# NonStopEagle137/Visual-Inertial-Odometry-MSCKF-Stereo

Measured on AMD Instinct MI355X. Metric: EKF measurement updates/sec at 30 cam-states x 200 features; ATE RMSE vs ref, higher is better.
Workload: dtype f32/f64; 1 GPU; batched EKF measurement update, 30 cam-states x 200 features, 2048 filters/GPU, triangulation + jacobian + gating + information assembly + Kalman, no row cap; cam_states=30, features=200, filters_per_gpu=2048, parallelism=replicas1

## Files before the change

visual-inertial-odometry-msckf-stereo_amd/csrc/msckf_api.hip:

```cpp
#include <hip/hip_runtime.h>

#include <algorithm>
#include <cmath>
#include <cstdio>
#include <cstring>
#include <string>
#include <vector>

#include "../../include/msckf_hip.h"
#include "msckf_common.h"
#include "msckf_launch.h"
#include "msckf_subbatch.h"

using namespace msckf;

static thread_local std::string g_err;

#define FAIL(code, ...)                                  \
    do {                                                 \
        char _b[512];                                    \
        snprintf(_b, sizeof(_b), __VA_ARGS__);           \
        g_err = _b;                                      \
        return (code);                                   \
    } while (0)
// ... 152 lines not shown
namespace {

template <typename T>
Params<T> make_params(const msckf_ctx* c) {
    Params<T> p{};
    const msckf_config_t& k = c->cfg;
    p.sigma2 = (T)k.observation_noise;
    p.qc_gyro = (T)k.gyro_noise;
    p.qc_gbias = (T)k.gyro_bias_noise;
    p.qc_acc = (T)k.acc_noise;
    p.qc_abias = (T)k.acc_bias_noise;
    for (int i = 0; i < 9; ++i) p.R01[i] = (T)k.R_cam0_cam1[i];
    for (int i = 0; i < 3; ++i) p.t01[i] = (T)k.t_cam0_cam1[i];
    p.huber = (T)k.huber_epsilon;
    p.precision = (T)k.estimation_precision;
    p.damping = (T)k.initial_damping;
    p.outer_max = k.outer_loop_max_iteration;
    p.inner_max = k.inner_loop_max_iteration;
    return p;
}

template <typename T>
DevState<T> dev_state(msckf_ctx* c, int b0 = 0, int nb = -1) {
    DevState<T> s;
    s.P = reinterpret_cast<T*>(c->P.p) + (size_t)b0 * c->Dmax * c->Dmax;
    s.imu = reinterpret_cast<T*>(c->imu.p) + (size_t)b0 * IMU_STRIDE;
    s.cams = reinterpret_cast<T*>(c->cams.p) + (size_t)b0 * c->Nmax * CAM_STRIDE;
    s.ncams = c->ncams.p + b0;
    s.B = nb < 0 ? c->B - b0 : nb;
    s.Nmax = c->Nmax;
    s.Dmax = c->Dmax;
    return s;
}

template <typename T>
UpdWs<T> upd_ws(msckf_ctx* c, int b0 = 0) {
    UpdWs<T> w;
    const size_t b = (size_t)b0, C = (size_t)c->Cmax;
    w.Cmax = c->Cmax;
    w.Cp = (c->Cmax + 15) & ~15;
    w.wk_stride = kalman_global_ws_doubles(c->Cmax);
    w.Hthin = reinterpret_cast<KT*>(c->Hthin.p) + b * C * (C + 1);
    w.dx = reinterpret_cast<KT*>(c->dx.p) + b * (c->Dmax + C);
    w.info = c->info.p + 4 * b;
    w.Lc = reinterpret_cast<KT*>(c->Lc.p) + b * w.Cp * w.Cp;
    w.afail = c->afail.p + b;
    w.Vi = reinterpret_cast<KT*>(c->Vi.p) + b * 24 * w.Cp;
    w.Sii = reinterpret_cast<KT*>(c->Sii.p) + b * 24 * 24;
    w.G = reinterpret_cast<KT*>(c->G.p) + b * C * (C + 1);
    w.Tm = reinterpret_cast<KT*>(c->Tm.p) + b * C * (C + 1);
    w.W = reinterpret_cast<KT*>(c->W.p) + b * (c->Dmax + 1) * w.Cp;
    w.Wk = c->Wk.p ? reinterpret_cast<KT*>(c->Wk.p) + b * w.wk_stride : nullptr;
    w.s2 = (double)(T)c->cfg.observation_noise;
    return w;
}

template <typename T>
FeatBatch<T> feat_batch(msckf_ctx* c) {
    FeatBatch<T> f;
    f.nf = c->nf;
    f.feat_filter = c->feat_filter;
    f.feat_off = c->feat_off;
    f.obs_off = c->obs_off;
    f.obs_cam = c->obs_cam;
    f.obs_z = reinterpret_cast<const T*>(c->obs_z);
    f.chi2 = reinterpret_cast<const T*>(c->chi2);
    f.ysq_off = c->ysq_off;
    f.p_w = reinterpret_cast<T*>(c->p_w);
    f.valid = c->valid;
    f.obs_ws = reinterpret_cast<T*>(c->obs_ws.p);
    f.obs_ht = reinterpret_cast<T*>(c->obs_ht.p);
    f.obs_g = reinterpret_cast<double*>(c->obs_g.p);
    f.fqr = reinterpret_cast<double*>(c->fqr.p);
    f.gram = c->gram ? 1 : 0;
    f.compact = feature_needs_compact(c->maxM) ? 1 : 0;
    f.tau = reinterpret_cast<T*>(c->tau.p);
    f.ysq = reinterpret_cast<T*>(c->ysq.p);
    f.gamma = reinterpret_cast<T*>(c->gamma);
    f.accept = c->accept;
    f.include = c->include;
    f.row_off = c->row_off.p;
    return f;
}

template <typename T>
std::vector<T> to_T(const double* x, size_t n) {
    std::vector<T> v(n);
    for (size_t i = 0; i < n; ++i) v[i] = (T)x[i];
    return v;
}

template <typename T>
hipError_t upload(msckf_ctx* c, void* dst, const double* src, size_t n) {
    if (n == 0) return hipSuccess;
    unsigned char* h = nullptr;
    hipError_t e = c->up.get(n * sizeof(T), &h);
    if (e != hipSuccess) return e;
    T* v = reinterpret_cast<T*>(h);
    for (size_t i = 0; i < n; ++i) v[i] = (T)src[i];
    e = hipMemcpyAsync(dst, h, n * sizeof(T), hipMemcpyHostToDevice, c->stream);
    if (e != hipSuccess) return e;
    return c->up.mark(c->stream);
}

hipError_t upload_raw(msckf_ctx* c, void* dst, const void* src, size_t bytes) {
    if (bytes == 0) return hipSuccess;
// ... 1089 lines not shown
        t->reset();
    }
    return 0;
}

int msckf_set_profiling_stage(msckf_ctx_t* c, const char* stage) {
    if (!c) FAIL(-1, "null context");
    if (int r = sync_lanes(c)) return r;
    for (KernelTimer* t : {&c->timer, &c->timer1}) {
        t->on = stage != nullptr;
        t->only = stage ? stage : "";
        t->reset();
    }
    return 0;
}

int msckf_kernel_times(msckf_ctx_t* c, int max_k, double* ms_total, int32_t* launches, char* names_out,
                       int names_cap) {
    if (!c) FAIL(-1, "null context");
    if (int r = sync_lanes(c)) return r;
    int k = std::min<int>(max_k, (int)c->timer.names.size());
    std::string all;
    for (int i = 0; i < k; ++i) {
        ms_total[i] = c->timer.total_ms[i];
        for (size_t j = 0; j < c->timer1.names.size(); ++j)
            if (c->timer1.names[j] == c->timer.names[i]) ms_total[i] += c->timer1.total_ms[j];
        launches[i] = c->timer.launches[i];
        all += c->timer.names[i];
        all.push_back('\0');
    }
    if (names_out && names_cap > 0) {
        int n = std::min<int>(names_cap - 1, (int)all.size());
        std::memcpy(names_out, all.data(), n);
        names_out[n] = 0;
    }
    return k;
}

int msckf_debug_workspace(msckf_ctx_t* c, int which, double* out, size_t count) {
    if (!c || !out) FAIL(-1, "null argument");
    JOIN_LANES(c);
    const void* src = which == 0 ? c->Lc.p : which == 1 ? c->Vi.p : which == 2 ? c->Sii.p
                    : which == 3 ? c->G.p : which == 4 ? c->Tm.p : which == 5 ? c->W.p
                    : which == 6 ? (const void*)c->Hthin.p : which == 7 ? (const void*)c->afail.p : nullptr;
    if (!src) FAIL(-1, "unknown workspace %d", which);
    HIPSYNC(c, hipStreamSynchronize(c->stream));
    HIPC(hipMemcpy(out, src, count * sizeof(double), hipMemcpyDeviceToHost));
    return 0;
}

int msckf_debug_set_workspace(msckf_ctx_t* c, int which, const double* in, size_t count) {
    if (!c || !in) FAIL(-1, "null argument");
    JOIN_LANES(c);
    void* dst = which == 6 ? (void*)c->Hthin.p : nullptr;
    if (!dst) FAIL(-1, "unknown workspace %d", which);
    if (count * sizeof(double) > c->Hthin.cap) FAIL(-1, "%zu doubles exceed H_thin", count);
    HIPSYNC(c, hipStreamSynchronize(c->stream));
    HIPC(hipMemcpy(dst, in, count * sizeof(double), hipMemcpyHostToDevice));
    return 0;
}

int msckf_debug_lanes(msckf_ctx_t* c) {
    if (!c) FAIL(-1, "null context");
    return c->last_lanes;
}

int msckf_debug_kalman(msckf_ctx_t* c) {
    if (c) c->last_async = "msckf_debug_kalman";
    if (!c) FAIL(-1, "null context");
    JOIN_LANES(c);
    return DISPATCH(c, run_kalman_only, c);
}

}
```

visual-inertial-odometry-msckf-stereo_amd/csrc/msckf_common.h:

```cpp
#pragma once
#include <hip/hip_runtime.h>
#include <stdint.h>

namespace msckf {

constexpr int IMU_STRIDE = 48;
enum ImuField { I_Q = 0, I_P = 4, I_V = 7, I_BG = 10, I_BA = 13, I_QN = 16, I_PN = 20,
                I_VN = 23, I_RIC = 26, I_TCI = 35, I_G = 38, I_ALIAS = 41 };
constexpr int CAM_STRIDE = 12;
enum CamField { C_Q = 0, C_P = 4, C_QN = 7 };

constexpr int OBS_HX = 0, OBS_V = 24, OBS_W = 36, OBS_QR = 54, OBS_R = 58, OBS_WS = 62;
constexpr int OBS_HT = 0, OBS_RT = 18, OBS_HTS = 24;

constexpr int OBG_G = 0, OBG_DS = 18, OBG_UB = 39, OBG_CAM = 45, OBG_STRIDE = 46;
constexpr int FQR_X = 0, FQR_G = 6, FQR_FLAG = 9, FQR_STRIDE = 10;
constexpr double FQR_RMAX = 1e3, FQR_KAPPA = 1e4;

template <typename T>
struct Params {
    T sigma2;
    T qc_gyro, qc_gbias, qc_acc, qc_abias;
    T R01[9], t01[3];
    T huber, precision, damping;
// ... 2 lines not shown

template <typename T>
struct DevState {
    T* P;
    T* imu;
    T* cams;
    int* ncams;
    int B, Nmax, Dmax;
};

template <typename T>
struct FeatBatch {
    int nf;
    const int* feat_filter;
    const int* feat_off;
    const int* obs_off;
    const int* obs_cam;
    const T* obs_z;
    const T* chi2;
    const long long* ysq_off;
    T* p_w;
    uint8_t* valid;
    T* obs_ws;
    T* obs_ht;
    double* obs_g;
    double* fqr;
    int gram;
    int compact;
    T* tau;
    T* ysq;
    T* gamma;
    uint8_t* accept;
    uint8_t* include;
    int* row_off;
};

using KT = double;
template <typename T>
struct UpdWs {
    KT* Hthin;
    KT* dx;
    int* info;
    int Cmax;
    KT* Lc;
    KT* Vi;
    KT* Sii;
    KT* G;
    KT* Tm;
    KT* W;
    KT* Wk;
    int* afail;
    size_t wk_stride;
    int Cp;
    double s2;
};

template <typename T> __device__ __forceinline__ T dsqrt(T x) { return sqrt(x); }

template <typename T>
__device__ __forceinline__ void skew3(const T* v, T* S) {
    S[0] = 0;     S[1] = -v[2]; S[2] = v[1];
    S[3] = v[2];  S[4] = 0;     S[5] = -v[0];
    S[6] = -v[1]; S[7] = v[0];  S[8] = 0;
}

template <typename T>
__device__ __forceinline__ void quat_to_rot(const T* q_in, T* R) {
    T n = sqrt(q_in[0] * q_in[0] + q_in[1] * q_in[1] + q_in[2] * q_in[2] + q_in[3] * q_in[3]);
    T x = q_in[0] / n, y = q_in[1] / n, z = q_in[2] / n, w = q_in[3] / n;
    T v[3] = {x, y, z};
    T S[9];
    skew3(v, S);
    T a = 2 * w * w - 1, tw = 2 * w;
#pragma unroll
    for (int i = 0; i < 3; ++i)
#pragma unroll
        for (int j = 0; j < 3; ++j)
            R[3 * i + j] = (i == j ? a : T(0)) - tw * S[3 * i + j] + (2 * v[i]) * v[j];
}

template <typename T>
__device__ __forceinline__ void rot_to_quat(const T* R, T* q) {
    T t;
    if (R[8] < 0) {
        if (R[0] > R[4]) {
            t = 1 + R[0] - R[4] - R[8];
            q[0] = t; q[1] = R[1] + R[3]; q[2] = R[6] + R[2]; q[3] = R[5] - R[7];
        } else {
            t = 1 - R[0] + R[4] - R[8];
            q[0] = R[1] + R[3]; q[1] = t; q[2] = R[7] + R[5]; q[3] = R[6] - R[2];
        }
    } else {
        if (R[0] < -R[4]) {
            t = 1 - R[0] - R[4] + R[8];
            q[0] = R[2] + R[6]; q[1] = R[7] + R[5]; q[2] = t; q[3] = R[1] - R[3];
        } else {
            t = 1 + R[0] + R[4] + R[8];
            q[0] = R[5] - R[7]; q[1] = R[6] - R[2]; q[2] = R[1] - R[3]; q[3] = t;
        }
    }
    T n = sqrt(q[0] * q[0] + q[1] * q[1] + q[2] * q[2] + q[3] * q[3]);
    q[0] /= n; q[1] /= n; q[2] /= n; q[3] /= n;
}

template <typename T>
__device__ __forceinline__ void quat_mul(const T* a_in, const T* b_in, T* q) {
// ... 111 lines not shown
```

visual-inertial-odometry-msckf-stereo_amd/csrc/msckf_kalman.hip:

```cpp
#include "msckf_common.h"
#include "msckf_launch.h"
#include "msckf_rchol.h"

#include <stdlib.h>

namespace msckf {

constexpr int KW = 24;

__device__ __forceinline__ int round4(int x) { return (x + 3) & ~3; }


typedef double v4d __attribute__((ext_vector_type(4)));

constexpr double KALMAN_PIVOT_FLOOR = 1e-10;

template <typename T>
__device__ double diag_max(const T* M, int ld, int o, int n, double* lds) {
    double m = 0.0;
    for (int i = threadIdx.x; i < n; i += blockDim.x) m = fmax(m, (double)M[(size_t)(o + i) * (ld + 1)]);
    m = wave_max(m);
    if ((threadIdx.x & 63) == 0) lds[threadIdx.x >> 6] = m;
    __syncthreads();
    for (int w = 0; w < (int)(blockDim.x >> 6); ++w) m = fmax(m, lds[w]);
// ... 5 lines not shown
    return diag_max(P, ld, 21, C, lds) * KALMAN_PIVOT_FLOOR;
}
constexpr double T_FLOOR_NEG = 1e-9;

template <typename T, int NT, int TPL, bool RETRY = false>
__global__ void __launch_bounds__(NT) __attribute__((amdgpu_waves_per_eu(NT == 256 ? 2 : 1))) k_kal_a(DevState<T> st, UpdWs<T> ws) {
    extern __shared__ __attribute__((aligned(16))) unsigned char smem_raw[];
    const int b = blockIdx.x;
    if (RETRY && ws.afail[b] == 0) return;
    const int C = 6 * st.ncams[b], Cp = round4(C);
    const int nrow = (Cp + KW) / 4;
    const T* P = st.P + (size_t)b * st.Dmax * st.Dmax;
    const int ld = st.Dmax, Cpw = ws.Cp;
    KT* Lc = ws.Lc + (size_t)b * Cpw * Cpw;
    KT* Vi = ws.Vi + (size_t)b * KW * Cpw;
    KT* Sii = ws.Sii + (size_t)b * KW * KW;
    auto map = [&](int i) { return i < C ? 21 + i : (i < Cp ? -1 : (i < Cp + 21 ? i - Cp : -1)); };
    double shift = 0.0;
    auto load = [&](int i, int j) -> double {
        const int mi = map(i), mj = map(j);
        if (mi < 0 || mj < 0) return i == j ? 1.0 : 0.0;
        return (double)P[(size_t)mi * ld + mj] + (i == j && i < C ? shift : 0.0);
    };
    auto panel = [&](int r, int c0, double w0, double w1, double w2, double w3) {
        KT* dst = r < Cp ? Lc + (size_t)r * Cpw + c0 : Vi + (size_t)(r - Cp) * Cpw + c0;
        dst[0] = w0; dst[1] = w1; dst[2] = w2; dst[3] = w3;
    };
    auto trail = [&](int i, int j, double v) { Sii[(i - Cp) * KW + (j - Cp)] = v; };
    const double floor = pcc_pivot_floor(P, ld, C, reinterpret_cast<double*>(smem_raw));
    bool ok = false;
    for (int att = RETRY ? 1 : 0; att < (RETRY ? 3 : 1) && !ok; ++att) {
        if (att > 0) {
            shift = (att == 1 ? 1e-8 : 1e-6) * (floor / KALMAN_PIVOT_FLOOR);
            __syncthreads();
        }
        ok = rchol_core<NT, TPL>(nrow, nrow, Cp / 4, reinterpret_cast<double*>(smem_raw), load, panel, trail, floor);
    }
    if (threadIdx.x == 0) ws.afail[b] = ok ? 0 : 1;
}

template <typename T, int NT, int TPL>
__global__ void __launch_bounds__(NT) __attribute__((amdgpu_waves_per_eu(NT == 256 ? 2 : 1))) k_kal_c1(DevState<T> st, UpdWs<T> ws) {
    extern __shared__ __attribute__((aligned(16))) unsigned char smem_raw[];
    const int b = blockIdx.x;
    if (ws.info[4 * b] == 0) return;
    if (ws.afail[b]) {
        if (threadIdx.x == 0) ws.info[4 * b + 3] = -2;
        return;
    }
    const int C = 6 * st.ncams[b], Cp = round4(C), nTc = Cp / 4;
    const int ldt = ws.Cmax + 1;
    const KT* Tm = ws.Tm + (size_t)b * ws.Cmax * ldt;
    KT* L = ws.G + (size_t)b * ws.Cmax * ldt;
    auto load = [&](int i, int j) -> double {
        if (i >= C || j >= C) return i == j ? 1.0 : 0.0;
        return i >= j ? Tm[(size_t)i * ldt + j] : Tm[(size_t)j * ldt + i];
    };
    auto panel = [&](int r, int c0, double w0, double w1, double w2, double w3) {
        if (r >= C) return;
        KT* dst = L + (size_t)r * ldt;
        const double w[4] = {w0, w1, w2, w3};
#pragma unroll
        for (int q = 0; q < 4; ++q)
            if (c0 + q < C && c0 + q <= r) dst[c0 + q] = w[q];
    };
    auto trail = [](int, int, double) {};
    const double tmax = diag_max(Tm, ldt, 0, C, reinterpret_cast<double*>(smem_raw));
    const bool ok = rchol_core<NT, TPL>(nTc, nTc, nTc, reinterpret_cast<double*>(smem_raw), load, panel, trail, ws.s2,
                                        -T_FLOOR_NEG * tmax);
    if (!ok && threadIdx.x == 0) ws.info[4 * b + 3] = -1;
}

constexpr int C2S = 17;

template <typename T, int NW, int CT, int NTM>
__global__ void __launch_bounds__(64 * NW) k_kal_c2(DevState<T> st, UpdWs<T> ws) {
    extern __shared__ __attribute__((aligned(16))) unsigned char smem_raw[];
    constexpr int NT = 64 * NW;
    const int b = blockIdx.x;
    if (ws.info[4 * b] == 0 || ws.info[4 * b + 3] < 0) return;
    const int C = 6 * st.ncams[b], nT = (C + 15) / 16, E = 22 + C, nE = (E + 15) / 16;
    const int tid = threadIdx.x, lane = tid & 63, lc = lane & 15, lr = lane >> 4;
    const int wv = __builtin_amdgcn_readfirstlane(tid >> 6);
    const int ldt = ws.Cmax + 1, Cpw = ws.Cp, ldw = st.Dmax + 1;
    const KT* L = ws.G + (size_t)b * ws.Cmax * ldt;
    const KT* Tm = ws.Tm + (size_t)b * ws.Cmax * ldt;
    const KT* Lc = ws.Lc + (size_t)b * Cpw * Cpw;
    const KT* Vi = ws.Vi + (size_t)b * KW * Cpw;
    KT* Wt = ws.W + (size_t)b * (st.Dmax + 1) * Cpw;
    double* LI = reinterpret_cast<double*>(smem_raw);
    double* img = LI + NTM * 256;
    auto Lv = [&](int r, int k) -> double {
        if (r >= C || k >= C) return r == k ? 1.0 : 0.0;
        return k <= r ? L[(size_t)r * ldt + k] : 0.0;
    };
    for (int J = wv; J < nT; J += NW) {
        double* blk = img + wv * 272;
#pragma unroll
        for (int q = 0; q < 4; ++q) {
            const int e = lane + 64 * q, i = e >> 4, k = e & 15;
            blk[e] = Lv(16 * J + i, 16 * J + k);
        }
        __builtin_amdgcn_wave_barrier();
        __builtin_amdgcn_fence(__ATOMIC_ACQ_REL, "wavefront");
        if (lane < 16) blk[256 + lane] = 1.0 / blk[17 * lane];
        __builtin_amdgcn_wave_barrier();
        __builtin_amdgcn_fence(__ATOMIC_ACQ_REL, "wavefront");
        if (lane < 16) {
            double x[16];
#pragma unroll
            for (int i = 0; i < 16; ++i) {
                double sv = i == lane ? 1.0 : 0.0;
#pragma unroll
                for (int k = 0; k < i; ++k) sv -= k >= lane ? blk[16 * i + k] * x[k] : 0.0;
                x[i] = i < lane ? 0.0 : sv * blk[256 + i];
            }
            double* xj = LI + J * 256 + 16 * lane;
#pragma unroll
            for (int i = 0; i < 16; ++i) xj[i] = x[i];
        }
        __builtin_amdgcn_wave_barrier();
        __builtin_amdgcn_fence(__ATOMIC_ACQ_REL, "wavefront");
    }
    auto Xv = [&](int e, int j) -> double {
        if (j >= C) return 0.0;
        if (e < 21) return Vi[(size_t)e * Cpw + j];
        if (e < 21 + C) return j <= e - 21 ? Lc[(size_t)(e - 21) * Cpw + j] : 0.0;
        if (e == 21 + C) return Tm[(size_t)j * ldt + C];
        return 0.0;
    };
    v4d yk[CT][NTM];
    constexpr int PFN = (256 * (NTM - 1) + NT - 1) / NT;
    double pf[PFN];
    auto fetch = [&](int J) {
        const int w = 16 * J;
#pragma unroll
        for (int q = 0; q < PFN; ++q) {
            const int e = tid + NT * q, i = e / w, col = e - i * w;
            pf[q] = e < 16 * w ? -Lv(16 * J + i, col) : 0.0;
        }
    };
    constexpr int IMGB = 16 * NTM * C2S;
    auto imgJ = [&](int J) { return img + (J & 1) * IMGB; };
    auto put = [&](int J) {
        const int w = 16 * J;
        double* im = imgJ(J);
#pragma unroll
        for (int q = 0; q < PFN; ++q) {
            const int e = tid + NT * q, i = e / w, col = e - i * w;
            if (e < 16 * w) im[col * C2S + i] = pf[q];
        }
    };
    __syncthreads();
    if (nT > 1) fetch(1);
    v4d xn[CT];
#pragma unroll
    for (int t = 0; t < CT; ++t) {
        const int ct = wv + NW * t;
#pragma unroll
        for (int q = 0; q < 4; ++q) xn[t][q] = ct < nE ? Xv(16 * ct + lc, lr + 4 * q) : 0.0;
    }
#pragma unroll
    for (int J = 0; J < NTM; ++J) {
        if (J >= nT) continue;
        if (J > 0) put(J);
        __syncthreads();
        if (J + 1 < nT) fetch(J + 1);
#pragma unroll
        for (int t = 0; t < CT; ++t) {
            const int ct = wv + NW * t;
            if (ct >= nE) continue;
            v4d a0 = xn[t], a1 = v4d{0.0, 0.0, 0.0, 0.0};
            if (J + 1 < nT) {
#pragma unroll
                for (int q = 0; q < 4; ++q) xn[t][q] = Xv(16 * ct + lc, 16 * (J + 1) + lr + 4 * q);
            }
            const double* im = imgJ(J);
#pragma unroll
            for (int K = 0; K < J; ++K) {
#pragma unroll
                for (int kc = 0; kc < 4; ++kc) {
                    const double av = im[(16 * K + 4 * kc + lr) * C2S + lc];
                    if (K & 1) a1 = __builtin_amdgcn_mfma_f64_16x16x4f64(av, yk[t][K][kc], a1, 0, 0, 0);
                    else a0 = __builtin_amdgcn_mfma_f64_16x16x4f64(av, yk[t][K][kc], a0, 0, 0, 0);
                }
            }
            a0 += a1;
            v4d y = v4d{0.0, 0.0, 0.0, 0.0};
#pragma unroll
            for (int kc = 0; kc < 4; ++kc)
                y = __builtin_amdgcn_mfma_f64_16x16x4f64(LI[J * 256 + (4 * kc + lr) * 16 + lc], a0[kc], y, 0, 0, 0);
            yk[t][J] = y;
        }
    }
#pragma unroll
    for (int t = 0; t < CT; ++t) {
        const int ct = wv + NW * t, col = 16 * ct + lc;
        if (ct >= nE || col >= E) continue;
#pragma unroll
        for (int J = 0; J < NTM; ++J) {
            if (J >= nT) continue;
#pragma unroll
            for (int q = 0; q < 4; ++q) {
                const int k = 16 * J + lr + 4 * q;
                if (k < C) Wt[(size_t)k * ldw + col] = yk[t][J][q];
            }
        }
    }
}

constexpr int GNB = 64;

__host__ __device__ constexpr size_t gchol_c_off(int Cmax) { return (size_t)(Cmax + 21) * (Cmax + 21); }
template <int STAGE, typename T>
__device__ __forceinline__ bool gdims(const DevState<T>& st, const UpdWs<T>& ws, int b, KT*& A, int& nrow,
                                      int& ncol, int& nelim) {
    if (ws.info[4 * b] == 0 || ws.info[4 * b + 3] < 0) return false;
    const int C = 6 * st.ncams[b];
    A = ws.Wk + (size_t)b * ws.wk_stride + (STAGE == 0 ? 0 : gchol_c_off(ws.Cmax));
    if (STAGE == 0) { nrow = C + 21; ncol = C + 21; }
    else { nrow = C + 22 + C; ncol = C; }
    nelim = C;
    return true;
}

template <int STAGE, typename T>
__global__ void __launch_bounds__(64) k_gchol_diag(DevState<T> st, UpdWs<T> ws, int k) {
    const int b = blockIdx.x;
    KT* A;
    int nrow, ncol, nelim;
    if (!gdims<STAGE>(st, ws, b, A, nrow, ncol, nelim) || k >= nelim) return;
    const int ld = ncol, nb = nelim - k < GNB ? nelim - k : GNB;
    __shared__ double colj[2][GNB];
    __shared__ double lt[GNB * (GNB + 1) / 2];
    const int lane = threadIdx.x;
    double x[GNB];
    {
        const KT* src = A + (size_t)(k + lane) * ld + k;
#pragma unroll
        for (int j = 0; j < GNB; ++j) x[j] = (lane < nb && j <= lane) ? src[j] : (j == lane ? 1.0 : 0.0);
    }
    double floor = STAGE == 0 ? 0.0 : ws.s2, lo;
    if (STAGE == 0) {
        const T* P = st.P + (size_t)b * st.Dmax * st.Dmax;
        for (int i = lane; i < nelim; i += 64) floor = fmax(floor, (double)P[(size_t)(21 + i) * st.Dmax + 21 + i]);
        floor = wave_max(floor) * KALMAN_PIVOT_FLOOR;
        lo = -PIVOT_FLOOR_NEG * floor;
    } else {
        const int ldt = ws.Cmax + 1;
        const KT* Tm = ws.Tm + (size_t)b * ws.Cmax * ldt;
        double tmax = 0.0;
        for (int i = lane; i < nelim; i += 64) tmax = fmax(tmax, (double)Tm[(size_t)i * ldt + i]);
        lo = -T_FLOOR_NEG * wave_max(tmax);
    }
// ... 438 lines not shown
            if (ti[s] < 0) continue;
#pragma unroll
            for (int r = 0; r < 4; ++r) {
                const int i = 16 * ti[s] + lr + 4 * r, j = 16 * tj[s] + lc;
                if (i < C && j <= i) Tm[(size_t)i * ld + j] = acc[s][r] + (i == j ? s2 : 0.0);
            }
        }
        if (tid < C) Tm[(size_t)tid * ld + C] = ca;
    }
}

template <typename T>
__global__ void __launch_bounds__(256) __attribute__((amdgpu_waves_per_eu(2))) k_kal_e(DevState<T> st, Params<T> prm, UpdWs<T> ws) {
    constexpr int TE = 128;
    const Blk3 bk = xcd_blk3();
    const int b = bk.z;
    if (ws.info[4 * b] == 0 || ws.info[4 * b + 3] < 0) return;
    const int C = 6 * st.ncams[b], D = 21 + C;
    const int i0 = bk.y * TE, j0 = bk.x * TE;
    if (i0 >= D || j0 > D) return;
    if (j0 > i0 + TE - 1 && !(D >= j0 && D < j0 + TE)) return;
    const int ld = st.Dmax;
    const KT* W = ws.Wk + (size_t)b * ws.wk_stride + gchol_c_off(ws.Cmax) + (size_t)C * C;
    const KT* Sii = ws.Sii + (size_t)b * KW * KW;
    T* P = st.P + (size_t)b * st.Dmax * st.Dmax;
    KT* dx = ws.dx + (size_t)b * (st.Dmax + ws.Cmax);
    const double s2 = (double)prm.sigma2;
    gemm_tile<TE, true, true>(D, D + 1, 0, C, i0, j0, [&](int i, int k) { return W[(size_t)i * C + k]; },
                       [&](int k, int j) { return W[(size_t)(j < D ? j : D) * C + k]; },
                       [&](int i, int j, double v) {
                           if (j < D && j <= i) {
                               double p = s2 * v;
                               if (i < 21 && j < 21) p += Sii[i * KW + j];
                               P[(size_t)i * ld + j] = (T)p;
                               P[(size_t)j * ld + i] = (T)p;
                           }
                           if (j == D) dx[i] = v;
                       });
}

template <typename T, int NW, int TPW>
__global__ void __launch_bounds__(64 * NW) k_kal_e1(DevState<T> st, Params<T> prm, UpdWs<T> ws) {
    extern __shared__ __attribute__((aligned(16))) unsigned char smem_raw[];
    const int b = blockIdx.x;
    if (ws.info[4 * b] == 0 || ws.info[4 * b + 3] < 0) return;
    const int C = 6 * st.ncams[b], D = 21 + C, nT = (D + 15) / 16, Dp = 16 * nT;
    const int tid = threadIdx.x, lane = tid & 63, lc = lane & 15, lr = lane >> 4;
    const int wv = __builtin_amdgcn_readfirstlane(tid >> 6);
    const int ntiles = nT * (nT + 1) / 2;
    const int Cpw = ws.Cp, ld = st.Dmax;
    const KT* W = ws.W + (size_t)b * (st.Dmax + 1) * Cpw;
    double* img = reinterpret_cast<double*>(smem_raw);
    double* yb = img + 2 * 16 * Dp;
    int ti[TPW], tj[TPW];
#pragma unroll
    for (int s = 0; s < TPW; ++s) {
        const int t = wv + NW * s;
        int i = (int)((sqrtf(8.0f * (float)t + 1.0f) - 1.0f) * 0.5f);
        while (i * (i + 1) / 2 > t) --i;
        while ((i + 1) * (i + 2) / 2 <= t) ++i;
        ti[s] = __builtin_amdgcn_readfirstlane(t < ntiles ? i : -1);
        tj[s] = __builtin_amdgcn_readfirstlane(t - i * (i + 1) / 2);
    }
    v4d acc[TPW];
#pragma unroll
    for (int s = 0; s < TPW; ++s) acc[s] = v4d{0.0, 0.0, 0.0, 0.0};
    double dxa = 0.0, dxb = 0.0;
    constexpr int NT = 64 * NW, Q = (16 * 16 * (NW * TPW <= 96 ? 13 : 15) + NT - 1) / NT;
    double rw[Q], ry = 0.0;
    const int ldw = st.Dmax + 1;
    auto load = [&](int k0) {
#pragma unroll
        for (int q = 0; q < Q; ++q) {
            const int e = tid + NT * q;
            const int k = e / Dp, row = e - k * Dp;
            rw[q] = (e < 16 * Dp && row < D && k0 + k < C) ? W[(size_t)(k0 + k) * ldw + row] : 0.0;
        }
        if (tid < 16) ry = k0 + tid < C ? W[(size_t)(k0 + tid) * ldw + D] : 0.0;
    };
    auto put = [&](int buf) {
        double* im = img + buf * 16 * Dp;
#pragma unroll
        for (int q = 0; q < Q; ++q) {
            const int e = tid + NT * q;
            if (e < 16 * Dp) im[e] = rw[q];
        }
        if (tid < 16) yb[buf * 16 + tid] = ry;
    };
    load(0);
    put(0);
    __syncthreads();
    for (int k0 = 0, it = 0; k0 < C; k0 += 16, ++it) {
        const int buf = it & 1;
        const bool more = k0 + 16 < C;
        if (more) load(k0 + 16);
        const double* im = img + buf * 16 * Dp;
#pragma unroll
        for (int kc = 0; kc < 4; ++kc) {
            const double* kr = im + (4 * kc + lr) * Dp;
#pragma unroll
            for (int s = 0; s < TPW; ++s) {
                if (ti[s] < 0) continue;
                acc[s] = __builtin_amdgcn_mfma_f64_16x16x4f64(kr[16 * ti[s] + lc], kr[16 * tj[s] + lc], acc[s], 0, 0, 0);
            }
        }
        if (tid < D) {
#pragma unroll
            for (int k = 0; k < 16; ++k) dxa += im[k * Dp + tid] * yb[buf * 16 + k];
        }
        if (NT + tid < D) {
#pragma unroll
            for (int k = 0; k < 16; ++k) dxb += im[k * Dp + NT + tid] * yb[buf * 16 + k];
        }
        if (more) put(buf ^ 1);
        __syncthreads();
    }
    const double s2 = (double)prm.sigma2;
    const KT* Sii = ws.Sii + (size_t)b * KW * KW;
    T* P = st.P + (size_t)b * st.Dmax * st.Dmax;
#pragma unroll
    for (int s = 0; s < TPW; ++s) {
        if (ti[s] < 0) continue;
#pragma unroll
        for (int r = 0; r < 4; ++r) {
            const int i = 16 * ti[s] + lr + 4 * r, j = 16 * tj[s] + lc;
            if (i >= D || j >= D || j > i) continue;
            double p = s2 * acc[s][r];
            if (i < 21 && j < 21) p += Sii[i * KW + j];
            P[(size_t)i * ld + j] = (T)p;
            P[(size_t)j * ld + i] = (T)p;
        }
    }
    if (tid < D) ws.dx[(size_t)b * (st.Dmax + ws.Cmax) + tid] = dxa;
    if (NT + tid < D) ws.dx[(size_t)b * (st.Dmax + ws.Cmax) + NT + tid] = dxb;
}

constexpr int MK_PS = 4;

__device__ __forceinline__ double mk_rcp(double x) {
    const double r = __builtin_amdgcn_rcp(x);
    return r * fma(-x, r, 2.0);
}

__host__ __device__ constexpr int mk_lds_doubles(int NBR) { return 2 * 16 * NBR * MK_PS + 16; }

template <typename T, int NW, int NBR, int STAGE>
__device__ __forceinline__ bool mk_factor(const DevState<T>& st, const UpdWs<T>& ws, int b, double shift,
                                          double floor, double lo, double* pan0) {
    constexpr int NBLK = NBR * (NBR + 1) / 2, SL = (NBLK + NW - 1) / NW;
    const int tid = threadIdx.x, lane = tid & 63, lc = lane & 15, lr = lane >> 4;
    const int wv = __builtin_amdgcn_readfirstlane(tid >> 6);
    const int C = 6 * st.ncams[b], Cp = round4(C);
    const int nrows = STAGE == 0 ? Cp + KW : C;
    const int nsteps = Cp / 4;
    const int ld = st.Dmax, Cpw = ws.Cp, ldt = ws.Cmax + 1;
    const T* P = st.P + (size_t)b * st.Dmax * st.Dmax;
    KT* Lc = ws.Lc + (size_t)b * Cpw * Cpw;
    KT* Vi = ws.Vi + (size_t)b * KW * Cpw;
    KT* Sii = ws.Sii + (size_t)b * KW * KW;
    const KT* Tm = ws.Tm + (size_t)b * ws.Cmax * ldt;
    KT* LT = ws.G + (size_t)b * ws.Cmax * ldt;
    auto map = [&](int i) { return i < C ? 21 + i : (i < Cp ? -1 : (i < Cp + 21 ? i - Cp : -1)); };
    auto load = [&](int i, int j) -> double {
        if (STAGE == 0) {
            const int mi = map(i), mj = map(j);
            if (mi < 0 || mj < 0) return i == j ? 1.0 : 0.0;
            return (double)P[(size_t)mi * ld + mj] + (i == j && i < C ? shift : 0.0);
        } else {
            if (i >= C || j >= C) return i == j ? 1.0 : 0.0;
            return i >= j ? Tm[(size_t)i * ldt + j] : Tm[(size_t)j * ldt + i];
        }
    };
    int brow[SL], bcol[SL];
#pragma unroll
    for (int j = 0; j < SL; ++j) {
        const int t = wv + NW * j;
        int cb = 0, rem = t;
        while (cb < NBR && rem >= NBR - cb) { rem -= NBR - cb; ++cb; }
        brow[j] = t < NBLK ? cb + rem : -1;
        bcol[j] = t < NBLK ? cb : NBR;
    }
    using v4d_t = double __attribute__((ext_vector_type(4)));
    v4d_t acc[SL];
#pragma unroll
    for (int j = 0; j < SL; ++j)
#pragma unroll
        for (int q = 0; q < 4; ++q)
            acc[j][q] = brow[j] >= 0 ? load(16 * brow[j] + lr + 4 * q, 16 * bcol[j] + lc) : 0.0;
    const double oh[4] = {lr == 0 ? 1.0 : 0.0, lr == 1 ? 1.0 : 0.0, lr == 2 ? 1.0 : 0.0, lr == 3 ? 1.0 : 0.0};
    for (int s = 0; s < nsteps; ++s) {
        const int KB = s >> 2, sc = s & 3, p0 = 4 * s;
        double* pan = pan0 + (s & 1) * 16 * NBR * MK_PS;
        if ((lc >> 2) == sc) {
#pragma unroll
            for (int j = 0; j < SL; ++j) {
                if (bcol[j] != KB) continue;
                double* d = pan + (16 * brow[j] + lr) * MK_PS + (lc & 3);
#pragma unroll
                for (int q = 0; q < 4; ++q) d[4 * q * MK_PS] = acc[j][q];
            }
        }
        __syncthreads();
        const double* ad = pan + p0 * MK_PS;
        const double a10 = ad[4], a20 = ad[8], a30 = ad[12];
        const double a21 = ad[9], a31 = ad[13], a32 = ad[14];
        const double d0 = pivot_floored(ad[0], floor, lo), e0 = mk_rcp(d0);
        const double l10 = a10 * e0, l20 = a20 * e0, l30 = a30 * e0;
        const double d1 = pivot_floored(ad[5] - l10 * a10, floor, lo), e1 = mk_rcp(d1);
        const double m21 = a21 - l20 * a10, m31 = a31 - l30 * a10;
        const double l21 = m21 * e1, l31 = m31 * e1;
        const double d2 = pivot_floored(ad[10] - l20 * a20 - l21 * m21, floor, lo), e2 = mk_rcp(d2);
        const double m32 = a32 - l30 * a20 - l31 * m21;
        const double l32 = m32 * e2;
        const double d3 = pivot_floored(ad[15] - l30 * a30 - l31 * m31 - l32 * m32, floor, lo), e3 = mk_rcp(d3);
        if (!(d0 > 0.0) || !(d1 > 0.0) || !(d2 > 0.0) || !(d3 > 0.0)) {
            __syncthreads();
            return false;
        }
        {
            const int r = p0 + tid;
            if (r < nrows) {
                const double* x = pan + r * MK_PS;
                const double z0 = x[0], z1 = x[1] - l10 * z0, z2 = x[2] - l20 * z0 - l21 * z1;
// ... 151 lines not shown

bool kalman_chol_supported(int Cmax) { return ((Cmax + 15) & ~15) <= 16 * 12; }

template <typename T, int NW, int TPW>
static void launch_e1(hipStream_t s, const DevState<T>& st, const Params<T>& prm, const UpdWs<T>& ws, size_t lds) {
    lds_limit((const void*)k_kal_e1<T, NW, TPW>, 160 * 1024);
    hipLaunchKernelGGL((k_kal_e1<T, NW, TPW>), dim3(st.B), dim3(64 * NW), lds, s, st, prm, ws);
}

template <typename T, int NT, int TPL>
static void launch_c1(hipStream_t s, const DevState<T>& st, const UpdWs<T>& ws, size_t lds) {
    hipLaunchKernelGGL((k_kal_c1<T, NT, TPL>), dim3(st.B), dim3(NT), lds, s, st, ws);
}
template <typename T, int NW, int CT, int NTM>
static void launch_c2(hipStream_t s, const DevState<T>& st, const UpdWs<T>& ws) {
    constexpr int IMG = 16 * NTM * C2S > NW * 272 ? 16 * NTM * C2S : NW * 272;
    const size_t lds = (NTM * 256 + 16 * NTM * C2S + IMG) * sizeof(double);
    lds_limit((const void*)k_kal_c2<T, NW, CT, NTM>, 160 * 1024);
    hipLaunchKernelGGL((k_kal_c2<T, NW, CT, NTM>), dim3(st.B), dim3(64 * NW), lds, s, st, ws);
}

template <typename T, int NW, int NTM>
static void launch_b(hipStream_t s, const DevState<T>& st, const Params<T>& prm, const UpdWs<T>& ws, size_t lds) {
    lds_limit((const void*)k_kal_b<T, NW, NTM>, 160 * 1024);
    hipLaunchKernelGGL((k_kal_b<T, NW, NTM>), dim3(st.B), dim3(64 * NW), lds, s, st, prm, ws);
}

template <typename T, int STAGE, int NBR>
static void launch_mk_nbr(hipStream_t s, const DevState<T>& st, const UpdWs<T>& ws) {
    constexpr int NW = 4;
    const size_t lds = mk_lds_doubles(NBR) * sizeof(double);
    hipLaunchKernelGGL((k_kal_mchol<T, NW, NBR, STAGE>), dim3(st.B), dim3(64 * NW), lds, s, st, ws);
    if constexpr (STAGE == 0)
        hipLaunchKernelGGL((k_kal_mchol<T, NW, NBR, STAGE, true>), dim3(st.B < 64 ? st.B : 64), dim3(64 * NW), lds, s,
                           st, ws);
}
template <typename T, int STAGE>
static void launch_mk(hipStream_t s, const DevState<T>& st, const UpdWs<T>& ws, int nbr) {
    if (nbr <= 8) launch_mk_nbr<T, STAGE, 8>(s, st, ws);
    else if (nbr <= 12) launch_mk_nbr<T, STAGE, 12>(s, st, ws);
    else if (nbr <= 13) launch_mk_nbr<T, STAGE, 13>(s, st, ws);
    else launch_mk_nbr<T, STAGE, 14>(s, st, ws);
}

constexpr int MK_MIN_B = 64;
static bool use_mk(int batch_B) {
    if (const char* e = getenv("MSCKF_KALMAN_CHOL")) {
        if (e[0] == 'm') return true;
        if (e[0] == 't') return false;
    }
    return batch_B >= MK_MIN_B;
}

template <typename T>
void launch_kalman_a_reg(hipStream_t s, const DevState<T>& st, const UpdWs<T>& ws, KernelTimer* kt, int batch_B) {
    if (st.B <= 0) return;
    const int Cp = (ws.Cmax + 3) & ~3;
    if (use_mk(batch_B)) {
        kt->begin(s, "kalman_a");
        launch_mk<T, 0>(s, st, ws, (Cp + KW + 15) / 16);
        kt->end(s);
        return;
    }
    const int nrow = (Cp + KW) / 4;
    RcholCfg c;
    pick_rchol(nrow * (nrow + 1) / 2, c);
    const size_t lds = rchol_lds_doubles(nrow) * sizeof(double);
    kt->begin(s, "kalman_a");
    if (c.nt == 256 && c.tpl == 4) launch_a_cfg<T, 256, 4>(s, st, ws, lds);
    else if (c.nt == 256) launch_a_cfg<T, 256, 6>(s, st, ws, lds);
    else launch_a_cfg<T, 512, 4>(s, st, ws, lds);
    kt->end(s);
}

template <typename T>
void launch_kalman_chol(hipStream_t s, const DevState<T>& st, const Params<T>& prm, const UpdWs<T>& ws,
                        KernelTimer* kt, int batch_B) {
    const int Cmax = ws.Cmax;
    const bool reg = kalman_chol_supported(Cmax);
    const int Cq = (Cmax + 15) & ~15;
    if (!reg) {
        kt->begin(s, "kalman_a");
        launch_gchol<0, T>(s, st, ws);
        kt->end(s);
    }
    kt->begin(s, "kalman_b");
    if (Cq <= 16 * 8) {
        launch_b<T, 8, 8>(s, st, prm, ws, (4 * 16 * (size_t)(Cq + 17) + 32) * sizeof(double));
    } else if (Cq <= 16 * 12) {
        launch_b<T, 16, 12>(s, st, prm, ws, (4 * 16 * (size_t)(Cq + 17) + 32) * sizeof(double));
    } else {
        const int tiles = (Cmax + GT - 1) / GT;
        hipLaunchKernelGGL(k_kal_b1<T>, dim3(tiles, tiles, st.B), dim3(256), 0, s, st, ws);
        hipLaunchKernelGGL(k_kal_b2<T>, dim3((Cmax + 1 + GT - 1) / GT, tiles, st.B), dim3(256), 0, s, st, prm, ws);
    }
    kt->end(s);
    kt->begin(s, "kalman_c");
    if (reg) {
        if (use_mk(batch_B)) {
            launch_mk<T, 1>(s, st, ws, (Cmax + 15) / 16);
        } else {
            const int nTc = ((Cmax + 3) & ~3) / 4;
            RcholCfg c;
            pick_rchol(nTc * (nTc + 1) / 2, c);
            const size_t lds = rchol_lds_doubles(nTc) * sizeof(double);
            if (c.nt == 256 && c.tpl == 4) launch_c1<T, 256, 4>(s, st, ws, lds);
// ... 34 lines not shown
```

visual-inertial-odometry-msckf-stereo_amd/csrc/msckf_launch.h:

```cpp
#pragma once
#include <hip/hip_runtime.h>

#include <mutex>
#include <string>
#include <utility>
#include <vector>

#include "msckf_common.h"
#include "msckf_gate_routes.h"

namespace msckf {

inline void lds_limit(const void* fn, size_t bytes) {
    if (bytes <= 64 * 1024) return;
    struct Grant { const void* fn; int dev; size_t bytes; };
    static std::mutex mu;
    static std::vector<Grant> grants;
    int dev = 0;
    (void)hipGetDevice(&dev);
    std::lock_guard<std::mutex> g(mu);
    for (auto& e : grants)
        if (e.fn == fn && e.dev == dev) {
            if (e.bytes >= bytes) return;
            (void)hipFuncSetAttribute(fn, hipFuncAttributeMaxDynamicSharedMemorySize, (int)bytes);
// ... 45 lines not shown
            pool.push_back(p.a);
            pool.push_back(p.b);
        }
        pending.clear();
    }
    void reset() { names.clear(); total_ms.clear(); launches.clear(); }
    ~KernelTimer() {
        for (auto& p : pending) { (void)hipEventDestroy(p.a); (void)hipEventDestroy(p.b); }
        for (auto e : pool) (void)hipEventDestroy(e);
    }
};

template <typename T>
void launch_propagate(hipStream_t, const DevState<T>&, const Params<T>&, int nfilt, const int* filters,
                      const int* smp_off, const T* samples);
template <typename T>
void launch_augment(hipStream_t, const DevState<T>&, int nfilt, const int* filters);
template <typename T>
void launch_prune(hipStream_t, const DevState<T>&, int nfilt, const int* filters, const int* keep_off,
                  const int* keep, const int* kcam_off, const int* keep_cams);
template <typename T>
void launch_cov_diag(hipStream_t, const DevState<T>&, int nfilt, const int* filters, int i0, int n, T* out);
struct SegClasses {
    static constexpr int NC = 5;
    static constexpr int S[NC] = {8, 16, 32, 64, 128};
    const int* list = nullptr;
    int off[NC + 1] = {};
    int beg[NC] = {}, end[NC] = {};
};
template <typename T>
void launch_triangulate(hipStream_t, const DevState<T>&, const Params<T>&, const FeatBatch<T>&, const SegClasses&);
template <typename T>
void launch_feature(hipStream_t, const DevState<T>&, const Params<T>&, const FeatBatch<T>&, const SegClasses&);
struct GateClasses {
    const int* list = nullptr;
    int off[GATE_NLIST + 1] = {};
    int beg[GATE_NLIST] = {}, end[GATE_NLIST] = {};
    int maxM[GATE_NLIST] = {};
};
template <typename T>
int launch_gate(hipStream_t, const DevState<T>&, const Params<T>&, const FeatBatch<T>&, const GateClasses&);
template <typename T>
bool launch_gate_tiles(hipStream_t, const DevState<T>&, const Params<T>&, const FeatBatch<T>&, const int* list,
                       int cnt, int nb, int maxM);
template <typename T>
void launch_select(hipStream_t, const DevState<T>&, const FeatBatch<T>&, const UpdWs<T>&, int row_cap);
template <typename T>
void launch_compress(hipStream_t, const DevState<T>&, const Params<T>&, const FeatBatch<T>&, const UpdWs<T>&, int maxnf,
                     int maxobs);
bool info_fused_fits(int Nmax, int maxnf);
inline bool feature_needs_compact(int maxM) { return maxM > GATE_TILE_MAXM; }
bool kalman_chol_supported(int Cmax);
size_t kalman_global_ws_doubles(int Cmax);
template <typename T>
void launch_kalman_a_reg(hipStream_t, const DevState<T>&, const UpdWs<T>&, KernelTimer*, int batch_B);
template <typename T>
void launch_kalman_chol(hipStream_t, const DevState<T>&, const Params<T>&, const UpdWs<T>&, KernelTimer*,
                        int batch_B);
template <typename T>
void launch_kalman(hipStream_t, const DevState<T>&, const Params<T>&, const UpdWs<T>&, KernelTimer*, int batch_B);

}
```

Measured before the change: 285,400 updates/s.

## Reverse camera ordering in Kalman Cholesky to skip structurally zero tiles

Adds a reversed camera-index ordering for the Kalman Cholesky factorization and the downstream triangular solves and Gram assembly, enabled by default for large batches or through an env var. With the reversed order, the triangular factor's structure puts leading blocks of the solve and the W-based Gram products at exact zeros. The kernels compute per-tile start indices, skip those zero MFMA tiles and prefetches, and force the corresponding W entries to zero. The goal is to cut wasted FLOPs in the tile loops. The cost is extra index arithmetic and a risk of subtle correctness problems in the ordering.

```diff
diff --git a/visual-inertial-odometry-msckf-stereo_amd/csrc/msckf_api.hip b/visual-inertial-odometry-msckf-stereo_amd/csrc/msckf_api.hip
--- a/visual-inertial-odometry-msckf-stereo_amd/csrc/msckf_api.hip
+++ b/visual-inertial-odometry-msckf-stereo_amd/csrc/msckf_api.hip
@@ -228,6 +228,7 @@
     w.W = reinterpret_cast<KT*>(c->W.p) + b * (c->Dmax + 1) * w.Cp;
     w.Wk = c->Wk.p ? reinterpret_cast<KT*>(c->Wk.p) + b * w.wk_stride : nullptr;
     w.s2 = (double)(T)c->cfg.observation_noise;
+    w.rev = kalman_reverse_order(c->B) ? 1 : 0;
     return w;
 }
 
@@ -1423,9 +1424,10 @@
 int msckf_debug_set_workspace(msckf_ctx_t* c, int which, const double* in, size_t count) {
     if (!c || !in) FAIL(-1, "null argument");
     JOIN_LANES(c);
-    void* dst = which == 6 ? (void*)c->Hthin.p : nullptr;
+    void* dst = which == 6 ? (void*)c->Hthin.p : which == 5 ? (void*)c->W.p : nullptr;
     if (!dst) FAIL(-1, "unknown workspace %d", which);
-    if (count * sizeof(double) > c->Hthin.cap) FAIL(-1, "%zu doubles exceed H_thin", count);
+    if (count * sizeof(double) > (which == 6 ? c->Hthin.cap : c->W.cap))
+        FAIL(-1, "%zu doubles exceed workspace %d", count, which);
     HIPSYNC(c, hipStreamSynchronize(c->stream));
     HIPC(hipMemcpy(dst, in, count * sizeof(double), hipMemcpyHostToDevice));
     return 0;
diff --git a/visual-inertial-odometry-msckf-stereo_amd/csrc/msckf_common.h b/visual-inertial-odometry-msckf-stereo_amd/csrc/msckf_common.h
--- a/visual-inertial-odometry-msckf-stereo_amd/csrc/msckf_common.h
+++ b/visual-inertial-odometry-msckf-stereo_amd/csrc/msckf_common.h
@@ -78,6 +78,7 @@
     int* afail;
     size_t wk_stride;
     int Cp;
+    int rev;
     double s2;
 };
 
diff --git a/visual-inertial-odometry-msckf-stereo_amd/csrc/msckf_kalman.hip b/visual-inertial-odometry-msckf-stereo_amd/csrc/msckf_kalman.hip
--- a/visual-inertial-odometry-msckf-stereo_amd/csrc/msckf_kalman.hip
+++ b/visual-inertial-odometry-msckf-stereo_amd/csrc/msckf_kalman.hip
@@ -81,9 +81,11 @@
     const int ldt = ws.Cmax + 1;
     const KT* Tm = ws.Tm + (size_t)b * ws.Cmax * ldt;
     KT* L = ws.G + (size_t)b * ws.Cmax * ldt;
+    const bool rev = ws.rev;
     auto load = [&](int i, int j) -> double {
         if (i >= C || j >= C) return i == j ? 1.0 : 0.0;
-        return i >= j ? Tm[(size_t)i * ldt + j] : Tm[(size_t)j * ldt + i];
+        const int ri = rev ? C - 1 - i : i, rj = rev ? C - 1 - j : j;
+        return ri >= rj ? Tm[(size_t)ri * ldt + rj] : Tm[(size_t)rj * ldt + ri];
     };
     auto panel = [&](int r, int c0, double w0, double w1, double w2, double w3) {
         if (r >= C) return;
@@ -151,14 +153,22 @@
         __builtin_amdgcn_wave_barrier();
         __builtin_amdgcn_fence(__ATOMIC_ACQ_REL, "wavefront");
     }
-    auto Xv = [&](int e, int j) -> double {
-        if (j >= C) return 0.0;
+    const bool rev = ws.rev;
+    auto Xv = [&](int e, int k) -> double {
+        if (k >= C) return 0.0;
+        const int j = rev ? C - 1 - k : k;
         if (e < 21) return Vi[(size_t)e * Cpw + j];
         if (e < 21 + C) return j <= e - 21 ? Lc[(size_t)(e - 21) * Cpw + j] : 0.0;
         if (e == 21 + C) return Tm[(size_t)j * ldt + C];
         return 0.0;
     };
     v4d yk[CT][NTM];
+    int J0[CT];
+#pragma unroll
+    for (int t = 0; t < CT; ++t) {
+        const int e0 = 16 * (wv + NW * t), e1 = e0 + 15;
+        J0[t] = __builtin_amdgcn_readfirstlane(rev && e0 >= 21 && e1 < 21 + C ? (C - 1 - (e1 - 21)) / 16 : 0);
+    }
     constexpr int PFN = (256 * (NTM - 1) + NT - 1) / NT;
     double pf[PFN];
     auto fetch = [&](int J) {
@@ -187,7 +197,7 @@
     for (int t = 0; t < CT; ++t) {
         const int ct = wv + NW * t;
 #pragma unroll
-        for (int q = 0; q < 4; ++q) xn[t][q] = ct < nE ? Xv(16 * ct + lc, lr + 4 * q) : 0.0;
+        for (int q = 0; q < 4; ++q) xn[t][q] = ct < nE && J0[t] == 0 ? Xv(16 * ct + lc, lr + 4 * q) : 0.0;
     }
 #pragma unroll
     for (int J = 0; J < NTM; ++J) {
@@ -200,13 +210,18 @@
             const int ct = wv + NW * t;
             if (ct >= nE) continue;
             v4d a0 = xn[t], a1 = v4d{0.0, 0.0, 0.0, 0.0};
-            if (J + 1 < nT) {
+            if (J + 1 < nT && J + 1 >= J0[t]) {
 #pragma unroll
                 for (int q = 0; q < 4; ++q) xn[t][q] = Xv(16 * ct + lc, 16 * (J + 1) + lr + 4 * q);
             }
+            if (J < J0[t]) {
+                yk[t][J] = a1;
+                continue;
+            }
             const double* im = imgJ(J);
 #pragma unroll
             for (int K = 0; K < J; ++K) {
+                if (K < J0[t]) continue;
 #pragma unroll
                 for (int kc = 0; kc < 4; ++kc) {
                     const double av = im[(16 * K + 4 * kc + lr) * C2S + lc];
@@ -228,7 +243,7 @@
         if (ct >= nE || col >= E) continue;
 #pragma unroll
         for (int J = 0; J < NTM; ++J) {
-            if (J >= nT) continue;
+            if (J >= nT || J < J0[t]) continue;
 #pragma unroll
             for (int q = 0; q < 4; ++q) {
                 const int k = 16 * J + lr + 4 * q;
@@ -773,15 +788,24 @@
     const KT* W = ws.W + (size_t)b * (st.Dmax + 1) * Cpw;
     double* img = reinterpret_cast<double*>(smem_raw);
     double* yb = img + 2 * 16 * Dp;
-    int ti[TPW], tj[TPW];
+    int ti[TPW], tj[TPW], kf[TPW];
 #pragma unroll
     for (int s = 0; s < TPW; ++s) {
         const int t = wv + NW * s;
-        int i = (int)((sqrtf(8.0f * (float)t + 1.0f) - 1.0f) * 0.5f);
-        while (i * (i + 1) / 2 > t) --i;
-        while ((i + 1) * (i + 2) / 2 <= t) ++i;
-        ti[s] = __builtin_amdgcn_readfirstlane(t < ntiles ? i : -1);
-        tj[s] = __builtin_amdgcn_readfirstlane(t - i * (i + 1) / 2);
+        int c = 0, rem = t;
+        if (rem >= nT) {
+            rem -= nT;
+            c = 1;
+            if (rem >= nT - 1) {
+                rem -= nT - 1;
+                c = nT - 1;
+                while (c > 1 && rem >= nT - c) { rem -= nT - c; --c; }
+            }
+        }
+        const int rmax = (16 * c + 15 < D ? 16 * c + 15 : D - 1) - 21;
+        ti[s] = __builtin_amdgcn_readfirstlane(t < ntiles ? c + rem : -1);
+        tj[s] = __builtin_amdgcn_readfirstlane(c);
+        kf[s] = __builtin_amdgcn_readfirstlane(ws.rev && c >= 2 ? (C - 1 - rmax) / 16 : 0);
     }
     v4d acc[TPW];
 #pragma unroll
@@ -794,8 +818,9 @@
 #pragma unroll
         for (int q = 0; q < Q; ++q) {
             const int e = tid + NT * q;
-            const int k = e / Dp, row = e - k * Dp;
-            rw[q] = (e < 16 * Dp && row < D && k0 + k < C) ? W[(size_t)(k0 + k) * ldw + row] : 0.0;
+            const int k = e / Dp, row = e - k * Dp, gk = k0 + k;
+            const bool zero = ws.rev && row >= 21 && gk + row - 21 < C - 1;
+            rw[q] = (e < 16 * Dp && row < D && gk < C && !zero) ? W[(size_t)gk * ldw + row] : 0.0;
         }
         if (tid < 16) ry = k0 + tid < C ? W[(size_t)(k0 + tid) * ldw + D] : 0.0;
     };
@@ -821,7 +846,7 @@
             const double* kr = im + (4 * kc + lr) * Dp;
 #pragma unroll
             for (int s = 0; s < TPW; ++s) {
-                if (ti[s] < 0) continue;
+                if (ti[s] < 0 || it < kf[s]) continue;
                 acc[s] = __builtin_amdgcn_mfma_f64_16x16x4f64(kr[16 * ti[s] + lc], kr[16 * tj[s] + lc], acc[s], 0, 0, 0);
             }
         }
@@ -889,7 +914,8 @@
             return (double)P[(size_t)mi * ld + mj] + (i == j && i < C ? shift : 0.0);
         } else {
             if (i >= C || j >= C) return i == j ? 1.0 : 0.0;
-            return i >= j ? Tm[(size_t)i * ldt + j] : Tm[(size_t)j * ldt + i];
+            const int ri = ws.rev ? C - 1 - i : i, rj = ws.rev ? C - 1 - j : j;
+            return ri >= rj ? Tm[(size_t)ri * ldt + rj] : Tm[(size_t)rj * ldt + ri];
         }
     };
     int brow[SL], bcol[SL];
@@ -1147,6 +1173,14 @@
     return batch_B >= MK_MIN_B;
 }
 
+bool kalman_reverse_order(int batch_B) {
+    if (const char* e = getenv("MSCKF_KALMAN_ORDER")) {
+        if (e[0] == 'r') return true;
+        if (e[0] == 'f') return false;
+    }
+    return batch_B >= MK_MIN_B;
+}
+
 template <typename T>
 void launch_kalman_a_reg(hipStream_t s, const DevState<T>& st, const UpdWs<T>& ws, KernelTimer* kt, int batch_B) {
     if (st.B <= 0) return;
diff --git a/visual-inertial-odometry-msckf-stereo_amd/csrc/msckf_launch.h b/visual-inertial-odometry-msckf-stereo_amd/csrc/msckf_launch.h
--- a/visual-inertial-odometry-msckf-stereo_amd/csrc/msckf_launch.h
+++ b/visual-inertial-odometry-msckf-stereo_amd/csrc/msckf_launch.h
@@ -121,6 +121,7 @@
 inline bool feature_needs_compact(int maxM) { return maxM > GATE_TILE_MAXM; }
 bool kalman_chol_supported(int Cmax);
 size_t kalman_global_ws_doubles(int Cmax);
+bool kalman_reverse_order(int batch_B);
 template <typename T>
 void launch_kalman_a_reg(hipStream_t, const DevState<T>&, const UpdWs<T>&, KernelTimer*, int batch_B);
 template <typename T>
```

After: 292,300 updates/s, median of 6. +2.4%, better.
